# ElementsProject/lightning

Measured on AMD Instinct MI355X. Metric: signature verifies/sec (ECDSA+Schnorr mix), higher is better.
Workload: dtype u32 (256-bit modular integer); 1 GPU; configs[1]+configs[2]: 1000000 ECDSA (65-byte keys, 65536 distinct) + 1000000 BIP-340 Schnorr per GPU per step, 90% valid / 10% invalid, inputs resident in HBM; parallelism=shard-by-row x1, RCCL all-gather of verdicts, key_table_cache=off (tables rebuilt every call)

## Files before the change

lightning_amd/csrc/engine_internal.h:

```cpp
#pragma once
#include <hip/hip_runtime.h>
#include <type_traits>
#include <stdio.h>
#include <stdlib.h>
#include <string.h>

#include <map>
#include <mutex>
#include <random>
#include <string>
#include <atomic>
#include <thread>
#include <vector>

#include "../../include/lightning_amd.h"
#include "../../include/lightning_amd_debug.h"
#include "verify_core.h"

using namespace lamd;

constexpr int MAX_LANES = 8;
#ifndef LAMD_PRIO_DEFAULT
#define LAMD_PRIO_DEFAULT 13
#endif
// ... 56 lines not shown
    for (auto &e : ev) {
      if (e) (void)hipEventDestroy(e);
      e = nullptr;
    }
  }
};

enum { Q_ECDSA33 = 0, Q_ECDSA65 = 1, Q_SCHNORR = 2, Q_KINDS = 3 };
#ifndef LAMD_QUEUE_SETS
#define LAMD_QUEUE_SETS 9
#endif
constexpr int QUEUE_SETS = LAMD_QUEUE_SETS;

struct lamd_ctx {
  int device = 0;
  int gtable_device = -1;
  hipStream_t stream = nullptr;
  hipDeviceProp_t prop;
  u32 *gtable = nullptr;
  std::string err;
  devbuf recs, qwords, keyok, slots, vbuf;
  devbuf row_ent, kd_table, kd_rep, kd_uid, kd_uniq, kd_count, kd_newent, plan, kt_fin;
  struct shape_ws { devbuf row, ent, slot, qwords, keyok, scratch; } hk[2];
  devbuf list7, list10, listcold, listcold_ok;
  u8 *h_small = nullptr;
  struct tmpl_ws {
    u8 *h = nullptr;
    size_t cap = 0;
  } tmpl;
  devbuf small_done;
  std::vector<u64> small_missed;
  u32 prio_mask = LAMD_PRIO_DEFAULT;
  unsigned spin_us = 2000;
  std::vector<u64> learn_fps;
  devbuf learn_dev;
  bool force_learn = false;
  u32 small_ticket = 0;
  bool small_kernel = true;
  u32 *h_plan = nullptr;
  struct key_cache {
    bool shared = false;
    u32 cap_ent = 0, cap7 = 0, cap10 = 0, index_mask = 0;
    devbuf ents, index, pool7, pool10, counters;
  } cache_store;
  key_cache *cache = nullptr;
  lamd_ctx *root = nullptr;
// ... 6 lines not shown
  int cache_mode = 1;
  size_t cache_keys = (size_t)1 << 20, cache_keys10 = (size_t)1 << 16;
  u32 cache_hwm[3] = {0, 0, 0};
  u32 cache_resets = 0;
  size_t last_hits = 0, last_cold = 0, last_l7 = 0, last_l10 = 0;
  devbuf keyok_row;
  hipStream_t stream2 = nullptr;
  hipStream_t stream3 = nullptr;
  hipEvent_t ev_fork = nullptr, ev_prep = nullptr, ev_cold = nullptr, ev_keys = nullptr, ev_sigs = nullptr;
  bool sigs_pending = false;
  hipEvent_t ev_sigs_wait = nullptr;
  static constexpr int MAX_COPY_STREAMS = 4;
  hipStream_t copy_streams[MAX_COPY_STREAMS] = {nullptr, nullptr, nullptr, nullptr};
  int n_copy_streams = 1;
  bool copy_one = true;
  int copy_events = 0;
  unsigned copy_turn = 0;
  bool use_copy_stream = true;
  int keyed_mode = -1;
  size_t keyed_min_rows = 8192;
  bool early_cold = true;
  bool fused_front = true;
  bool kc_tree = false;
  bool small_fused = true;
  bool last_small_fused = false;
  size_t last_small_n = 0;
  double keyed_min_uses = 6.0;
  double keyed_dense_uses = 48.0;
  int keyed_teeth = 0;
  int last_mode = 0;
  size_t last_n = 0;
  bool last_keyed_call = false;
  devbuf in_a, in_b, in_c, out;
  devbuf g_msgs, g_off, g_ids, g_rowbase, g_hash, g_sig, g_pub, g_malformed, g_ok, g_verdict;
  struct store_ws {
    devbuf img, host, ids, tab, out, rep, pack, dig, rng, rng_out, cmp, cmp_out, dir, sq, sq_out, ts, ts_msg, ts_out, rx, rx_out;
    stage_timer<6> t_audit;
    stage_timer<4> t_rep;
    stage_timer<6> t_dig;
    stage_timer<7> t_rx;
    void destroy_events() { t_audit.destroy(); t_rep.destroy(); t_dig.destroy(); t_rx.destroy(); }
  } store;
  struct text_ws {
    devbuf cols;
    stage_timer<3> t;
    double ms[2] = {0, 0};
// ... 101 lines not shown
```

lightning_amd/csrc/lamd_common.h:

```cpp
#pragma once
#include <stddef.h>
#include <stdint.h>

#if defined(__HIPCC__)
#include <hip/hip_runtime.h>
#define LAMD_HD __host__ __device__ __forceinline__
#define LAMD_HD_NOINLINE __host__ __device__ __noinline__
#else
#define LAMD_HD static inline __attribute__((always_inline))
#define LAMD_HD_NOINLINE static __attribute__((noinline))
#endif

#if defined(LAMD_CHECK_MAG)
#include <assert.h>
#define LAMD_ASSERT(x) assert(x)
#else
#define LAMD_ASSERT(x) ((void)0)
#endif

namespace lamd {
typedef uint32_t u32;
typedef uint64_t u64;
typedef uint8_t u8;
}
```

lightning_amd/csrc/lamd_engine.hip:

```cpp
#include "engine_internal.h"
#include "fuzz.h"
#include "host_ranges.h"
#include "key_column.h"
#include "table_audit.h"

using namespace lamd;

__device__ u32 g_prio;
#define LAMD_PRIO(bit)                                     \
  do {                                                     \
    if (g_prio & (bit)) __builtin_amdgcn_s_setprio(3);     \
  } while (0)


__global__ void __launch_bounds__(256) k_gtable_build(u32 *__restrict__ gtable, const u32 *__restrict__ bases) {
  const size_t idx = (size_t)blockIdx.x * blockDim.x + threadIdx.x;
  if (idx >= GTABLE_ENTRIES) return;
  const u32 w = (u32)(idx >> GTABLE_WINDOW_BITS), d = (u32)(idx & ((1u << GTABLE_WINDOW_BITS) - 1u));
  u32 out[GT_ENTRY_WORDS];
  if (d == 0) {
#pragma unroll
    for (int i = 0; i < GT_ENTRY_WORDS; i++) out[i] = 0;
  } else {
    u32 base[16];
// ... 484 lines not shown
#pragma unroll
  for (int i = 0; i < 8; i++) { qx[i] = qwords[u * 16 + i]; qy[i] = qwords[u * 16 + 8 + i]; }
  kc_prefix<T>(pool + (size_t)slots[u] * kc_stride(T), scratch + u * kc_scratch_words(T), ge_from_words(qx, qy));
}
template <int T>
__global__ void __launch_bounds__(256) k_kc_chain_bwd(const u32 *__restrict__ plan, int which, u32 cap, const u8 *__restrict__ keyok,
                                                      u32 *__restrict__ pool, const u32 *__restrict__ slots, const u32 *__restrict__ scratch) {
  const size_t t = (size_t)blockIdx.x * blockDim.x + threadIdx.x;
  const size_t u = t / kc_nsub(T);
  const u32 nkeys = plan[which] < cap ? plan[which] : cap;
  if (u >= nkeys || !keyok[u]) return;
  kc_chain_bwd<T>(pool + (size_t)slots[u] * kc_stride(T), scratch + u * kc_scratch_words(T), (int)(t % kc_nsub(T)));
}
struct kc_shape_args {
  u32 cap;
  const u32 *hk_row;
  const u32 *hk_ent, *hk_slot;
  u32 *qwords;
  u8 *keyok;
  u32 *scratch;
  u32 *pool;
};
template <int T>
static void launch_keytables(hipStream_t st, const u32 *plan, int which, const kc_shape_args &A) {
  const size_t cap = A.cap, chains = cap * kc_nsub(T);
  hipLaunchKernelGGL((k_kc_bases<T>), dim3((unsigned)((cap + 255) / 256)), dim3(256), 0, st, plan, which, A.cap, A.qwords, A.keyok, A.scratch);
  hipLaunchKernelGGL((k_kc_chain_fwd<T>), dim3((unsigned)((chains + 255) / 256)), dim3(256), 0, st, plan, which, A.cap, A.keyok, A.pool, A.hk_slot, A.scratch);
  hipLaunchKernelGGL((k_kc_prefix<T>), dim3((unsigned)((cap + 255) / 256)), dim3(256), 0, st, plan, which, A.cap, A.qwords, A.keyok, A.pool, A.hk_slot,
                     A.scratch);
  hipLaunchKernelGGL((k_kc_chain_bwd<T>), dim3((unsigned)((chains + 255) / 256)), dim3(256), 0, st, plan, which, A.cap, A.keyok, A.pool, A.hk_slot,
                     A.scratch);
}

template <int T>
__device__ __forceinline__ void keys_bases_body(size_t u, const u32 *__restrict__ plan, int which, const kc_shape_args &A, const u8 *__restrict__ keys,
                                                int keylen, size_t stride) {
  const u32 nkeys = plan[which] < A.cap ? plan[which] : A.cap;
  if (u >= nkeys) return;
  u32 qx[8], qy[8];
  const bool ok = parse_pubkey(keys + stride * (size_t)A.hk_row[u], keylen, qx, qy);
  uint4 *dst = reinterpret_cast<uint4 *>(A.qwords + u * 16);
  dst[0] = make_uint4(qx[0], qx[1], qx[2], qx[3]);
  dst[1] = make_uint4(qx[4], qx[5], qx[6], qx[7]);
  dst[2] = make_uint4(qy[0], qy[1], qy[2], qy[3]);
  dst[3] = make_uint4(qy[4], qy[5], qy[6], qy[7]);
  A.keyok[u] = ok;
  if (ok) kc_bases<T>(A.scratch + u * kc_scratch_words(T), ge_from_words(qx, qy));
}
__global__ void __launch_bounds__(256) k_keys_bases_both(const u32 *__restrict__ plan, unsigned blocks7, kc_shape_args A7, kc_shape_args A10,
                                                         const u8 *__restrict__ keys, int keylen, size_t stride) {
  LAMD_PRIO(8);
  if (blockIdx.x < blocks7) keys_bases_body<7>((size_t)blockIdx.x * blockDim.x + threadIdx.x, plan, P_HK7, A7, keys, keylen, stride);
  else keys_bases_body<10>((size_t)(blockIdx.x - blocks7) * blockDim.x + threadIdx.x, plan, P_HK10, A10, keys, keylen, stride);
}
struct publish_args {
  const u8 *keys;
  int keylen;
  size_t stride;
  u32 lane, seq;
  u64 seed;
  cache_ent *ents;
  u32 *index;
  u32 mask;
  int do_index;
};
template <int T>
__device__ __forceinline__ void kc_finish_body(size_t t, const u32 *__restrict__ plan, int which, const kc_shape_args &A, const publish_args &P) {
  constexpr int NS = kc_nsub(T);
  static_assert(256 % NS == 0, "a key's chains must not straddle blocks");
  const size_t u = t / NS;
  const int sub = (int)(t % NS);
  const u32 nkeys = plan[which] < A.cap ? plan[which] : A.cap;
  const bool live = u < nkeys;
  const bool ok = live && A.keyok[u];
  u32 *tab = ok ? A.pool + (size_t)A.hk_slot[u] * kc_stride(T) : nullptr;
  u32 *scr = A.scratch + u * kc_scratch_words(T);
  if (ok) kc_chain_fwd<T>(tab, scr, sub);
  __syncthreads();
  if (live && sub == 0) {
    if (ok) {
      u32 qx[8], qy[8];
#pragma unroll
      for (int i = 0; i < 8; i++) { qx[i] = A.qwords[u * 16 + i]; qy[i] = A.qwords[u * 16 + 8 + i]; }
      kc_prefix<T>(tab, scr, ge_from_words(qx, qy));
    }
    cache_ent e;
    key_words(e.kw, P.keys + P.stride * (size_t)A.hk_row[u], P.keylen);
    e.meta = (ok ? (u32)T : 0u) | (P.lane << 8);
    e.seq = P.seq;
    e.tabslot = A.hk_slot[u];
    const u32 id = A.hk_ent[u];
    P.ents[id] = e;
    if (P.do_index) {
      __threadfence();
      u32 slot = (u32)key_words_hash(e.kw, P.seed) & P.mask;
      for (;;) {
        if (atomicCAS(&P.index[slot], 0u, id + 1u) == 0u) break;
        slot = (slot + 1u) & P.mask;
      }
    }
  }
  __syncthreads();
  if (ok) kc_chain_bwd<T>(tab, scr, sub);
}
__global__ void __launch_bounds__(256) k_kc_finish_both(const u32 *__restrict__ plan, unsigned blocks7, kc_shape_args A7, kc_shape_args A10, publish_args P) {
  LAMD_PRIO(8);
  if (blockIdx.x < blocks7) kc_finish_body<7>((size_t)blockIdx.x * blockDim.x + threadIdx.x, plan, P_HK7, A7, P);
  else kc_finish_body<10>((size_t)(blockIdx.x - blocks7) * blockDim.x + threadIdx.x, plan, P_HK10, A10, P);
}

template <int T, int KPL>
__device__ __forceinline__ void kc_tree_body(size_t t, const u32 *__restrict__ plan, int which, const kc_shape_args &A, const publish_args &P) {
  const u32 nkeys = plan[which] < A.cap ? plan[which] : A.cap;
  const size_t u0 = t * KPL;
  if (u0 >= nkeys) return;
  kc_tree_keys K;
  ge qs[KPL];
  K.n = 0;
#pragma unroll 1
  for (int k = 0; k < KPL; k++) {
    const size_t u = u0 + k;
    if (u >= nkeys) break;
    const bool ok = A.keyok[u] != 0;
    if (ok) {
      u32 qx[8], qy[8];
#pragma unroll
      for (int i = 0; i < 8; i++) { qx[i] = A.qwords[u * 16 + i]; qy[i] = A.qwords[u * 16 + 8 + i]; }
      qs[K.n] = ge_from_words(qx, qy);
      K.tab[K.n] = A.pool + (size_t)A.hk_slot[u] * kc_stride(T);
      K.scr[K.n] = A.scratch + u * kc_scratch_words(T);
      K.n++;
// ... 412 lines not shown
    HIPCHK(ctx, hipDeviceSynchronize());
    HIPCHK(ctx, hipFree(b->p));
  }
  b->p = nullptr;
  b->cap = 0;
  size_t want = bytes + bytes / 4 + 4096;
  if (hipMalloc(&b->p, want) != hipSuccess) {
    want = bytes;
    hipError_t e = hipMalloc(&b->p, want);
    if (e != hipSuccess) {
      ctx->err = std::string("hipMalloc: ") + hipGetErrorString(e);
      return LAMD_ERR_NOMEM;
    }
  }
  b->cap = want;
  return LAMD_OK;
}

static unsigned careful_grid(const lamd_ctx *ctx, size_t n) {
  const bool flood = ctx->h_plan && ((volatile const u32 *)ctx->h_plan)[P_SUSPECT] > 4096u;
  return flood || blocks_for(n) < 64u ? blocks_for(n) : 64u;
}

static unsigned keyed_grid(size_t n) { return (unsigned)((n + KEYED_THREADS - 1) / KEYED_THREADS); }

static int hw_queues_from_env(void) {
  const char *v = getenv("GPU_MAX_HW_QUEUES");
  return v && *v ? atoi(v) : 0;
}

extern "C" const char *lamd_version(void) { return "lightning_amd 0.1 (gfx950)"; }

extern "C" const char *lamd_last_error(const lamd_ctx *ctx) { return ctx ? ctx->err.c_str() : "no context"; }

static int init_known_answers(lamd_ctx *ctx);
static int cache_alloc(lamd_ctx *owner, lamd_ctx::key_cache *kc, size_t keys7, size_t keys10, bool shared);
static int cache_reset(lamd_ctx *root);

static int create_streams(lamd_ctx *ctx) {
  HIPCHK(ctx, hipStreamCreateWithFlags(&ctx->stream, hipStreamNonBlocking));
  HIPCHK(ctx, hipStreamCreateWithFlags(&ctx->stream2, hipStreamNonBlocking));
  if (!getenv("LAMD_MERGE_SIDE") || atoi(getenv("LAMD_MERGE_SIDE")) != 0) ctx->stream3 = ctx->stream2;
  else HIPCHK(ctx, hipStreamCreateWithFlags(&ctx->stream3, hipStreamNonBlocking));
  HIPCHK(ctx, hipEventCreateWithFlags(&ctx->ev_cold, hipEventDisableTiming));
  HIPCHK(ctx, hipEventCreateWithFlags(&ctx->ev_keys, hipEventDisableTiming));
  HIPCHK(ctx, hipEventCreateWithFlags(&ctx->ev_sigs, hipEventDisableTiming));
// ... 82 lines not shown
  if (!out) return LAMD_ERR_ARG;
  *out = nullptr;
  int count = 0;
  if (hipGetDeviceCount(&count) != hipSuccess || count <= 0) return LAMD_ERR_NO_DEVICE;
  if (device < 0 || device >= count) return LAMD_ERR_ARG;
  lamd_ctx *ctx = new (std::nothrow) lamd_ctx();
  if (!ctx) return LAMD_ERR_NOMEM;
  ctx->device = device;
  *out = ctx;
  HIPCHK(ctx, hipSetDevice(device));
  HIPCHK(ctx, hipGetDeviceProperties(&ctx->prop, device));
  if (strncmp(ctx->prop.gcnArchName, "gfx950", 6) != 0) {
    ctx->err = std::string("unsupported architecture ") + ctx->prop.gcnArchName + " (built for gfx950 only)";
    return LAMD_ERR_NO_DEVICE;
  }
  if (const char *w = getenv("LAMD_ECMULT_WAVES")) ctx->ecmult_waves = atoi(w);
  if (const char *w = getenv("LAMD_PAIRS")) ctx->pairs = atoi(w) != 0;
  if (const char *w = getenv("LAMD_GROUP")) ctx->group_rows = atoi(w) != 0;
  if (const char *w = getenv("LAMD_SPIN_US")) ctx->spin_us = (unsigned)atoi(w);
  if (const char *w = getenv("LAMD_PRIO")) ctx->prio_mask = (u32)atoi(w);
  if (const char *w = getenv("LAMD_FUSED_FRONT")) ctx->fused_front = atoi(w) != 0;
  if (const char *w = getenv("LAMD_EARLY_COLD")) ctx->early_cold = atoi(w) != 0;
  if (const char *w = getenv("LAMD_KC_TREE")) ctx->kc_tree = atoi(w) != 0;
  if (const char *w = getenv("LAMD_PREP_BATCH")) ctx->prep_batch = atoi(w) < 1 ? 1 : (size_t)atoi(w);
  if (const char *w = getenv("LAMD_PREP_MIN_THREADS")) ctx->prep_min_threads = atol(w) < 0 ? 0 : (size_t)atol(w);
  {
    std::random_device rd;
    ctx->hash_seed = ((u64)rd() << 32) ^ (u64)rd() ^ 0x243F6A8885A308D3ULL;
  }
  if (const char *w = getenv("LAMD_CHUNK_ROWS")) ctx->chunk = (size_t)atoll(w) < 4 ? 4 : (size_t)atoll(w);
  if (const char *w = getenv("LAMD_KEYED")) ctx->keyed_mode = atoi(w);
  if (const char *w = getenv("LAMD_KEYED_MIN_USES")) ctx->keyed_min_uses = atof(w);
  if (const char *w = getenv("LAMD_KEYED_DENSE_USES")) ctx->keyed_dense_uses = atof(w);
  if (const char *w = getenv("LAMD_KEYED_TEETH")) ctx->keyed_teeth = atoi(w) == 7 ? 7 : (atoi(w) == 10 ? 10 : 0);
  if (const char *w = getenv("LAMD_KEYED_MIN_ROWS")) ctx->keyed_min_rows = (size_t)atoll(w);
  if (const char *w = getenv("LAMD_SMALL_FUSED")) ctx->small_fused = atoi(w) != 0;
  if (const char *w = getenv("LAMD_CACHE")) ctx->cache_mode = atoi(w) != 0;
  if (const char *w = getenv("LAMD_SMALL_KERNEL")) ctx->small_kernel = atoi(w) != 0;
  if (const char *w = getenv("LAMD_CACHE_KEYS")) ctx->cache_keys = (size_t)atoll(w) < 64 ? 64 : (size_t)atoll(w);
  if (const char *w = getenv("LAMD_CACHE_KEYS10")) ctx->cache_keys10 = (size_t)atoll(w) < 16 ? 16 : (size_t)atoll(w);
  int rc = create_streams(ctx);
  if (rc != LAMD_OK) return rc;
  std::vector<u32> bases(GTABLE_WINDOWS * 16);
  {
    const u32 gx[8] = LAMD_GX, gy[8] = LAMD_GY;
    u32 cur[16];
// ... 521 lines not shown
  const size_t n = c.n;
  lamd_ctx::key_cache *kc = f.kc;
  {
    const size_t words = f.m > n ? f.m : n;
    const unsigned ib = blocks_for(words / 4 + 1);
    hipLaunchKernelGGL(k_call_init, dim3(ib < 2048u ? ib : 2048u), dim3(256), 0, ctx->stream, f.plan, ctx->kd_table.as<u32>(), f.m, ctx->kd_count.as<u32>(), n,
                       f.use_cache ? (u32 *)nullptr : f.row_ent, f.use_cache ? (u32 *)nullptr : f.cc);
  }
  if (f.use_cache && (rc = launch_cache_lookup(ctx, root, c, f)) != LAMD_OK) return rc;
  hipLaunchKernelGGL(k_dedupe_insert_count, dim3(blocks_for(n)), dim3(256), 0, ctx->stream, n, c.d_key, c.keylen, c.keystride, root->hash_seed,
                     (const u32 *)f.row_ent, ctx->kd_table.as<u32>(), (u32)(f.m - 1), ctx->kd_rep.as<u32>(), f.plan, ctx->kd_uniq.as<u32>(), ctx->kd_count.as<u32>());
  launch_classify<true>(ctx, c, f);
  if (c.time_it) HIPCHK(ctx, hipEventRecord(ctx->ev[1], ctx->stream));
  if (ctx->early_cold) {
    hipLaunchKernelGGL(k_partition_cold, dim3(blocks_for(n)), dim3(256), 0, ctx->stream, n, ctx->kd_rep.as<const u32>(), ctx->kd_newent.as<const u32>(), f.plan,
                       f.listcold);
    if ((rc = launch_cold(ctx, c, f.listcold, f.plan, f.fin)) != LAMD_OK) return rc;
    *cold_started = true;
  }
  const bool on7 = f.thr[0] != NO_TABLES, on10 = f.thr[1] != NO_TABLES;
  if (on7 || on10) {
    const kc_shape_args A7 = shape_args(ctx->hk[0], on7 ? f.cap[0] : 0, kc->pool7), A10 = shape_args(ctx->hk[1], on10 ? f.cap[1] : 0, kc->pool10);
    const unsigned kb7 = on7 ? blocks_for(f.cap[0]) : 0u, kb10 = on10 ? blocks_for(f.cap[1]) : 0u;
    hipLaunchKernelGGL(k_keys_bases_both, dim3(kb7 + kb10), dim3(256), 0, ctx->stream, (const u32 *)f.plan, kb7, A7, A10, c.d_key, c.keylen, c.keystride);
    const publish_args P = {c.d_key, c.keylen, c.keystride, (u32)ctx->lane_id, f.seq ? f.seq : 1u, root->hash_seed, kc->ents.as<cache_ent>(), kc->index.as<u32>(),
                            kc->index_mask, (int)f.use_cache};
    if (root->kc_tree) {
      const unsigned tb7 = on7 ? (unsigned)((f.cap[0] + 64 * KC_TREE_KPL7 - 1) / (64 * KC_TREE_KPL7)) : 0u;
      const unsigned tb10 = on10 ? (unsigned)((f.cap[1] + 64 * KC_TREE_KPL10 - 1) / (64 * KC_TREE_KPL10)) : 0u;
      hipLaunchKernelGGL(k_kc_tree_both, dim3(tb7 + tb10), dim3(64), 0, ctx->stream, (const u32 *)f.plan, tb7, A7, A10, P);
    } else {
      const unsigned fb7 = on7 ? blocks_for(f.cap[0] * kc_nsub(7)) : 0u, fb10 = on10 ? blocks_for(f.cap[1] * kc_nsub(10)) : 0u;
      hipLaunchKernelGGL(k_kc_finish_both, dim3(fb7 + fb10), dim3(256), 0, ctx->stream, (const u32 *)f.plan, fb7, A7, A10, P);
    }
  }
  if ((rc = mark_published(ctx, root, f)) != LAMD_OK) return rc;
  auto part = *cold_started ? k_partition<true, true> : k_partition<true, false>;
  hipLaunchKernelGGL(part, dim3(blocks_for(n)), dim3(256), 0, ctx->stream, n, f.row_ent, ctx->kd_rep.as<const u32>(), (const u32 *)nullptr,
                     ctx->kd_newent.as<const u32>(), kc->ents.as<const cache_ent>(), f.plan, f.list7, f.list10, f.listcold, c.keyok_out, c.d_ok, c.d_sig, c.mode);
  return LAMD_OK;
}

static int front_end_legacy(lamd_ctx *ctx, lamd_ctx *root, const chunk_io &c, const front_args &f) {
  int rc;
  const size_t n = c.n;
  lamd_ctx::key_cache *kc = f.kc;
  HIPCHK(ctx, hipMemsetAsync(f.plan, 0, P_WORDS * 4, ctx->stream));
  HIPCHK(ctx, hipMemsetAsync(ctx->kd_table.p, 0, f.m * 4, ctx->stream));
  HIPCHK(ctx, hipMemsetAsync(ctx->kd_count.p, 0, n * 4, ctx->stream));
  if (f.use_cache) {
    if ((rc = launch_cache_lookup(ctx, root, c, f)) != LAMD_OK) return rc;
  } else {
    HIPCHK(ctx, hipMemsetAsync(f.row_ent, 0xFF, n * 4, ctx->stream));
    HIPCHK(ctx, hipMemsetAsync(f.cc, 0, C_WORDS * 4, ctx->stream));
  }
  hipLaunchKernelGGL(k_dedupe_insert, dim3(blocks_for(n)), dim3(256), 0, ctx->stream, n, c.d_key, c.keylen, c.keystride, root->hash_seed, (const u32 *)f.row_ent,
// ... 103 lines not shown
}

static int chunk_partitioned(lamd_ctx *ctx, lamd_ctx *root, const chunk_io &c, bool use_cache, bool small, bool latency_learn) {
  int rc;
  const size_t n = c.n;
  front_args f = {};
  f.use_cache = use_cache;
  table_thresholds(ctx, small, use_cache, latency_learn, f.thr);
  for (int s = 0; s < 2; s++) f.cap[s] = f.thr[s] == NO_TABLES ? 1 : n / f.thr[s] + 1;
  lamd_ctx::key_cache *kc = f.kc = use_cache ? &root->cache_store : &ctx->cache_store;
  if (!use_cache && (rc = cache_alloc(ctx, kc, f.cap[0], f.cap[1], false)) != LAMD_OK) return rc;
  f.m = 4;
  while (f.m < 2 * n) f.m <<= 1;
  if ((rc = ensure(ctx, &ctx->kd_table, f.m * 4)) != LAMD_OK) return rc;
  for (devbuf *b : {&ctx->row_ent, &ctx->kd_rep, &ctx->kd_uid, &ctx->kd_uniq, &ctx->kd_count, &ctx->kd_newent, &ctx->list7, &ctx->list10,
                    &ctx->listcold})
    if ((rc = ensure(ctx, b, n * 4)) != LAMD_OK) return rc;
  for (int s = 0; s < 2; s++) {
    lamd_ctx::shape_ws &w = ctx->hk[s];
    for (devbuf *b : {&w.row, &w.ent, &w.slot})
      if ((rc = ensure(ctx, b, f.cap[s] * 4)) != LAMD_OK) return rc;
    if ((rc = ensure(ctx, &w.qwords, f.cap[s] * 64)) != LAMD_OK) return rc;
    if ((rc = ensure(ctx, &w.keyok, f.cap[s])) != LAMD_OK) return rc;
    if ((rc = ensure(ctx, &w.scratch, f.cap[s] * kc_scratch_words(s ? 10 : 7) * 4)) != LAMD_OK) return rc;
  }
  if ((rc = ensure(ctx, &ctx->plan, P_WORDS * 4)) != LAMD_OK) return rc;
  if (c.mode == MODE_SCHNORR && (rc = ensure(ctx, &ctx->kt_fin, n * (size_t)FIN_WORDS * 4)) != LAMD_OK) return rc;
  f.plan = ctx->plan.as<u32>();
  f.cc = kc->counters.as<u32>();
  f.row_ent = ctx->row_ent.as<u32>();
  f.list7 = ctx->list7.as<u32>();
  f.list10 = ctx->list10.as<u32>();
  f.listcold = ctx->listcold.as<u32>();
  f.fin = c.mode == MODE_SCHNORR ? ctx->kt_fin.as<u32>() : nullptr;
  if (use_cache) {
    f.vis = cache_visibility(root, ctx);
    f.seq = ++root->call_seq;
  }
  f.lf = {nullptr, 0, c.d_key, c.keylen, c.keystride, root->hash_seed, 0xFFFFFFFFu, 0xFFFFFFFFu};
  if (small && use_cache) {
    f.lf.budget7 = kc->cap7 / 2;
    f.lf.budget10 = kc->cap10 / 2;
    if (latency_learn && !ctx->learn_fps.empty()) {
      const size_t nf = ctx->learn_fps.size() < 4096 ? ctx->learn_fps.size() : 4096;
      if ((rc = ensure(ctx, &ctx->learn_dev, nf * 8)) != LAMD_OK) return rc;
      HIPCHK(ctx, hipMemcpyAsync(ctx->learn_dev.p, ctx->learn_fps.data(), nf * 8, hipMemcpyHostToDevice, ctx->stream));
      f.lf.fps = ctx->learn_dev.as<const u64>();
// ... 1213 lines not shown
```

lightning_amd/csrc/verify_core.h:

```cpp
#pragma once
#include "group.h"
#include "scalar.h"
#include "sha256.h"

namespace lamd {

enum { MODE_ECDSA = 0, MODE_SCHNORR = 1, MODE_RECOVER = 2 };

#define LAMD_S30_P {0x3FFFFC2F, 0x3FFFFFFB, 0x3FFFFFFF, 0x3FFFFFFF, 0x3FFFFFFF, 0x3FFFFFFF, 0x3FFFFFFF, 0x3FFFFFFF, 0xFFFF}
LAMD_HD fe fe_inv_var(const fe &a) {
  const int32_t pl[9] = LAMD_S30_P;
  u32 aw[8], w[9];
  fe_to_words(aw, fe_normalize(a));
  s30_inverse(w, aw, pl, 0x2DDACACFu);
  const u32 p32[9] = {0xFFFF85E0u, 0xFFFFFFDFu, 0xFFFFFFFFu, 0xFFFFFFFFu, 0xFFFFFFFFu, 0xFFFFFFFFu, 0xFFFFFFFFu, 0xFFFFFFFFu, 0x1Fu};
  u64 cy = 0;
#pragma unroll
  for (int i = 0; i < 9; i++) {
    cy += (u64)w[i] + p32[i];
    w[i] = (u32)cy;
    cy >>= 32;
  }
  u32 q = w[8];
#pragma unroll
// ... 346 lines not shown
  const fe zi = fe_inv_var(acc.z);
  const fe zi2 = fe_sqr(zi);
  slot_store_fe(out, fe_mul(acc.x, zi2));
  slot_store_fe(out + TW, fe_mul(acc.y, fe_mul(zi2, zi)));
}

constexpr int kc_spacing(int T) { return T == 7 ? 19 : T == 8 ? 17 : T == 9 ? 15 : T == 10 ? 13 : 12; }
constexpr int kc_ne(int T) { return 1 << (T - 1); }
constexpr int KC_SUB_LOG = 4, KC_SUB = 1 << KC_SUB_LOG;
constexpr int kc_nsub(int T) { return kc_ne(T) / KC_SUB; }
constexpr int kc_words(int T) { return (kc_ne(T) + 1) * SLOT_ENTRY_WORDS; }
constexpr int kc_stride(int T) { return kc_words(T) + 16; }
constexpr int KC_P0 = 0, KC_ZB = 27, KC_C = 36;
constexpr int kc_sub_off(int T) { return KC_C + (T - 1) * 18; }
constexpr int KC_SUB_WORDS = 18 + (KC_SUB - 1) * 9;
constexpr int kc_scratch_words(int T) { return kc_sub_off(T) + kc_nsub(T) * KC_SUB_WORDS; }
static_assert(kc_nsub(7) * KC_SUB_WORDS >= 13 * 36 && kc_nsub(8) * KC_SUB_WORDS >= 15 * 36, "stage-1 parking space");

LAMD_HD void store_raw(u32 *dst, const fe &a) {
#pragma unroll
  for (int i = 0; i < 9; i++) dst[i] = a.n[i];
}

template <int T>
LAMD_HD void kc_bases(u32 *scratch, const ge &q) {
  constexpr int D = kc_spacing(T), NPT = 2 * T - 1;
  u32 *tmp = scratch + kc_sub_off(T);
  gej b = gej_from_ge(q);
#pragma unroll 1
  for (int i = 0; i < NPT; i++) {
    store_raw(tmp + i * 36 + 0, b.x);
    store_raw(tmp + i * 36 + 9, b.y);
    store_raw(tmp + i * 36 + 18, fe_norm_weak(b.z));
    if (i == NPT - 1) break;
    const int nd = (i & 1) ? D - 1 : 1;
#pragma unroll 1
    for (int j = 0; j < nd; j++) b = gej_double(b);
  }
  fe acc = fe_set_int(1);
#pragma unroll 1
  for (int i = 0; i < NPT; i++) {
    store_raw(tmp + i * 36 + 27, acc);
    acc = fe_mul(acc, slot_load_raw(tmp + i * 36 + 18));
  }
  store_raw(scratch + KC_ZB, acc);
  fe suffix = fe_set_int(1);
#pragma unroll 1
  for (int i = NPT - 1; i >= 0; i--) {
    const fe ratio = fe_mul(suffix, slot_load_raw(tmp + i * 36 + 27));
    suffix = fe_mul(suffix, slot_load_raw(tmp + i * 36 + 18));
    const fe r2 = fe_sqr(ratio);
    const fe x = fe_mul(slot_load_raw(tmp + i * 36 + 0), r2);
    const fe y = fe_mul(slot_load_raw(tmp + i * 36 + 9), fe_mul(r2, ratio));
    u32 *dst = (i & 1) ? scratch + KC_C + (i >> 1) * 18 : tmp + i * 36;
    store_raw(dst + 0, x);
    store_raw(dst + 9, y);
  }
  gej p;
  p.x = slot_load_raw(tmp + (NPT - 1) * 36 + 0);
  p.y = slot_load_raw(tmp + (NPT - 1) * 36 + 9);
  p.z = fe_set_int(1);
  p.inf = false;
#pragma unroll 1
  for (int i = 0; i < T - 1; i++) {
    ge m;
    m.x = slot_load_raw(tmp + 2 * i * 36 + 0);
    m.y = fe_norm_weak(fe_neg(slot_load_raw(tmp + 2 * i * 36 + 9), 1));
    bool degenerate;
    fe h, rr;
    p = gej_add_ge_core(p, m, &degenerate, &h, &rr);
  }
  store_raw(scratch + KC_P0 + 0, p.x);
  store_raw(scratch + KC_P0 + 9, p.y);
  store_raw(scratch + KC_P0 + 18, fe_norm_weak(p.z));
}
template <int T>
LAMD_HD void kc_chain_fwd(u32 *tab, u32 *scratch, int sub) {
  u32 *sp = scratch + kc_sub_off(T) + sub * KC_SUB_WORDS;
  u32 *ent = tab + sub * KC_SUB * SLOT_ENTRY_WORDS;
  gej p;
  p.x = slot_load_raw(scratch + KC_P0 + 0);
  p.y = slot_load_raw(scratch + KC_P0 + 9);
  p.z = slot_load_raw(scratch + KC_P0 + 18);
  p.inf = false;
  bool degenerate;
  fe h, rr;
#pragma unroll 1
  for (int b = 0; b < T - 1 - KC_SUB_LOG; b++) {
    if ((sub >> b) & 1) {
      ge c;
      c.x = slot_load_raw(scratch + KC_C + (KC_SUB_LOG + b) * 18 + 0);
      c.y = slot_load_raw(scratch + KC_C + (KC_SUB_LOG + b) * 18 + 9);
      p = gej_add_ge_core(p, c, &degenerate, &h, &rr);
      p.z = fe_norm_weak(p.z);
    }
  }
  slot_store_fe(ent + 0, p.x);
  slot_store_fe(ent + ENT_Y, p.y);
#pragma unroll 1
  for (int g = 1; g < KC_SUB; g++) {
    const int c = __builtin_ctz((unsigned)g), gr = g ^ (g >> 1);
    ge pt;
    pt.x = slot_load_raw(scratch + KC_C + c * 18 + 0);
    pt.y = slot_load_raw(scratch + KC_C + c * 18 + 9);
    pt = ge_neg_if(pt, ((gr >> c) & 1) == 0);
    p = gej_add_ge_core(p, pt, &degenerate, &h, &rr);
    slot_store_fe(ent + gr * SLOT_ENTRY_WORDS + 0, p.x);
    slot_store_fe(ent + gr * SLOT_ENTRY_WORDS + ENT_Y, p.y);
    store_raw(sp + 18 + (g - 1) * 9, h);
  }
  store_raw(sp + 0, fe_norm_weak(p.z));
}
template <int T>
LAMD_HD void kc_prefix(u32 *tab, u32 *scratch, const ge &q) {
  constexpr int NS = kc_nsub(T), NE = kc_ne(T);
  u32 *sp = scratch + kc_sub_off(T);
  fe acc = fe_set_int(1);
#pragma unroll 1
  for (int s = 0; s < NS; s++) {
    store_raw(sp + s * KC_SUB_WORDS + 9, acc);
    acc = fe_mul(acc, slot_load_raw(sp + s * KC_SUB_WORDS + 0));
  }
  const fe zc = fe_mul(acc, slot_load_raw(scratch + KC_ZB));
  slot_store_fe(tab + kc_words(T), zc);
  fe suffix = fe_set_int(1);
#pragma unroll 1
  for (int s = NS - 1; s >= 0; s--) {
    const fe ratio = fe_mul(suffix, slot_load_raw(sp + s * KC_SUB_WORDS + 9));
    suffix = fe_mul(suffix, slot_load_raw(sp + s * KC_SUB_WORDS + 0));
    store_raw(sp + s * KC_SUB_WORDS + 9, ratio);
  }
  const u32 betaw[8] = LAMD_BETA;
  const fe z2 = fe_sqr(zc);
  const fe x = fe_mul(q.x, z2);
  u32 *e = tab + NE * SLOT_ENTRY_WORDS;
  slot_store_fe(e + 0, x);
  slot_store_fe(e + ENT_BX, fe_mul(x, fe_from_words(betaw)));
  slot_store_fe(e + ENT_Y, fe_mul(q.y, fe_mul(z2, zc)));
}
template <int T>
LAMD_HD void kc_chain_bwd(u32 *tab, const u32 *scratch, int sub) {
  const u32 betaw[8] = LAMD_BETA;
  const fe beta = fe_from_words(betaw);
  const u32 *sp = scratch + kc_sub_off(T) + sub * KC_SUB_WORDS;
  u32 *ent = tab + sub * KC_SUB * SLOT_ENTRY_WORDS;
  fe rho = slot_load_raw(sp + 9);
#pragma unroll 1
  for (int g = KC_SUB - 1; g >= 0; g--) {
    if (g != KC_SUB - 1) rho = fe_mul(rho, slot_load_raw(sp + 18 + g * 9));
    const int gr = g ^ (g >> 1);
    const fe r2 = fe_sqr(rho);
    const fe x = fe_mul(slot_load_fe(ent + gr * SLOT_ENTRY_WORDS + 0), r2);
    const fe y = fe_mul(slot_load_fe(ent + gr * SLOT_ENTRY_WORDS + ENT_Y), fe_mul(r2, rho));
    slot_store_fe(ent + gr * SLOT_ENTRY_WORDS + 0, x);
    slot_store_fe(ent + gr * SLOT_ENTRY_WORDS + ENT_BX, fe_mul(x, beta));
    slot_store_fe(ent + gr * SLOT_ENTRY_WORDS + ENT_Y, y);
  }
}
template <int T>
LAMD_HD void keytable_build(u32 *tab, u32 *scratch, const ge &q) {
  kc_bases<T>(scratch, q);
  for (int s = 0; s < kc_nsub(T); s++) kc_chain_fwd<T>(tab, scratch, s);
  kc_prefix<T>(tab, scratch, q);
  for (int s = 0; s < kc_nsub(T); s++) kc_chain_bwd<T>(tab, scratch, s);
}

constexpr int KC_TREE_MAXK = 4;
struct kc_tree_keys {
  u32 *tab[KC_TREE_MAXK];
  u32 *scr[KC_TREE_MAXK];
  int n;
};
template <int T>
LAMD_HD void kc_tree_affine(const kc_tree_keys &K, const ge *qs) {
  constexpr int NE = kc_ne(T);
  static_assert(kc_nsub(T) * KC_SUB_WORDS >= (NE / 2) * 9, "prefix products of the last level fit the per-chain scratch");
  const u32 betaw[8] = LAMD_BETA;
  const fe beta = fe_from_words(betaw);
  fe acc = fe_set_int(1);
#pragma unroll 1
// ... 1352 lines not shown
```

Measured before the change: 248.7 million verifies/s.

## Interleave key-table scratch per lane and run table kernels as persistent grids

Key-table scratch moves from a flat per-key layout to a lane-interleaved layout of 16-byte chunks, so neighbouring threads' loads and stores coalesce. The chain kernel now parks intermediate points in a per-block chain buffer instead of writing them to the table and reading them back. Both table kernels become grid-stride loops over groups, sized by a grid that defaults to the CU count and can be set with LAMD_TABLE_GRID. The publish step also hashes key words while writing them in place. The catch is extra scratch memory and a bigger chunk footprint (9-word elements padded to 12), and the smaller grid may cut parallelism if one block per CU cannot hide latency.

```diff
diff --git a/lightning_amd/csrc/engine_internal.h b/lightning_amd/csrc/engine_internal.h
--- a/lightning_amd/csrc/engine_internal.h
+++ b/lightning_amd/csrc/engine_internal.h
@@ -102,6 +102,7 @@
   devbuf recs, qwords, keyok, slots, vbuf;
   devbuf row_ent, kd_table, kd_rep, kd_uid, kd_uniq, kd_count, kd_newent, plan, kt_fin;
   struct shape_ws { devbuf row, ent, slot, qwords, keyok, scratch; } hk[2];
+  devbuf kc_chains;
   devbuf list7, list10, listcold, listcold_ok;
   u8 *h_small = nullptr;
   struct tmpl_ws {
@@ -154,6 +155,7 @@
   bool early_cold = true;
   bool fused_front = true;
   bool kc_tree = false;
+  unsigned table_grid = 0;
   bool small_fused = true;
   bool last_small_fused = false;
   size_t last_small_n = 0;
diff --git a/lightning_amd/csrc/lamd_common.h b/lightning_amd/csrc/lamd_common.h
--- a/lightning_amd/csrc/lamd_common.h
+++ b/lightning_amd/csrc/lamd_common.h
@@ -6,9 +6,11 @@
 #include <hip/hip_runtime.h>
 #define LAMD_HD __host__ __device__ __forceinline__
 #define LAMD_HD_NOINLINE __host__ __device__ __noinline__
+#define LAMD_HD_MEMBER __host__ __device__ __forceinline__
 #else
 #define LAMD_HD static inline __attribute__((always_inline))
 #define LAMD_HD_NOINLINE static __attribute__((noinline))
+#define LAMD_HD_MEMBER inline __attribute__((always_inline))
 #endif
 
 #if defined(LAMD_CHECK_MAG)
diff --git a/lightning_amd/csrc/lamd_engine.hip b/lightning_amd/csrc/lamd_engine.hip
--- a/lightning_amd/csrc/lamd_engine.hip
+++ b/lightning_amd/csrc/lamd_engine.hip
@@ -530,6 +530,10 @@
   u32 *pool;
 };
 template <int T>
+__device__ __forceinline__ kc_lanes kc_key_view(u32 *scratch, size_t u) {
+  return kc_lanes{scratch + (u / 64u) * (size_t)(64 * 4 * kc_key_chunks(T)), 64, u % 64u};
+}
+template <int T>
 static void launch_keytables(hipStream_t st, const u32 *plan, int which, const kc_shape_args &A) {
   const size_t cap = A.cap, chains = cap * kc_nsub(T);
   hipLaunchKernelGGL((k_kc_bases<T>), dim3((unsigned)((cap + 255) / 256)), dim3(256), 0, st, plan, which, A.cap, A.qwords, A.keyok, A.scratch);
@@ -540,10 +544,8 @@
                      A.scratch);
 }
 
-template <int T>
-__device__ __forceinline__ void keys_bases_body(size_t u, const u32 *__restrict__ plan, int which, const kc_shape_args &A, const u8 *__restrict__ keys,
-                                                int keylen, size_t stride) {
-  const u32 nkeys = plan[which] < A.cap ? plan[which] : A.cap;
+template <int T, bool LANES>
+__device__ __forceinline__ void keys_bases_body(size_t u, u32 nkeys, const kc_shape_args &A, const u8 *__restrict__ keys, int keylen, size_t stride) {
   if (u >= nkeys) return;
   u32 qx[8], qy[8];
   const bool ok = parse_pubkey(keys + stride * (size_t)A.hk_row[u], keylen, qx, qy);
@@ -553,13 +555,22 @@
   dst[2] = make_uint4(qy[0], qy[1], qy[2], qy[3]);
   dst[3] = make_uint4(qy[4], qy[5], qy[6], qy[7]);
   A.keyok[u] = ok;
-  if (ok) kc_bases<T>(A.scratch + u * kc_scratch_words(T), ge_from_words(qx, qy));
-}
-__global__ void __launch_bounds__(256) k_keys_bases_both(const u32 *__restrict__ plan, unsigned blocks7, kc_shape_args A7, kc_shape_args A10,
-                                                         const u8 *__restrict__ keys, int keylen, size_t stride) {
+  if (!ok) return;
+  if constexpr (LANES) kc_bases_at<T>(kc_key_view<T>(A.scratch, u), ge_from_words(qx, qy));
+  else kc_bases<T>(A.scratch + u * kc_scratch_words(T), ge_from_words(qx, qy));
+}
+template <bool LANES>
+__global__ void __launch_bounds__(256) k_keys_bases_both(const u32 *__restrict__ plan, kc_shape_args A7, kc_shape_args A10, const u8 *__restrict__ keys,
+                                                         int keylen, size_t stride) {
   LAMD_PRIO(8);
-  if (blockIdx.x < blocks7) keys_bases_body<7>((size_t)blockIdx.x * blockDim.x + threadIdx.x, plan, P_HK7, A7, keys, keylen, stride);
-  else keys_bases_body<10>((size_t)(blockIdx.x - blocks7) * blockDim.x + threadIdx.x, plan, P_HK10, A10, keys, keylen, stride);
+  const u32 n7 = plan[P_HK7] < A7.cap ? plan[P_HK7] : A7.cap, n10 = plan[P_HK10] < A10.cap ? plan[P_HK10] : A10.cap;
+  const u32 groups7 = (n7 + 63u) / 64u, groups = groups7 + (n10 + 63u) / 64u;
+  const u32 lane = threadIdx.x & 63u, waves = gridDim.x * (blockDim.x / 64u);
+#pragma unroll 1
+  for (u32 g = blockIdx.x * (blockDim.x / 64u) + threadIdx.x / 64u; g < groups; g += waves) {
+    if (g < groups7) keys_bases_body<7, LANES>((size_t)g * 64u + lane, n7, A7, keys, keylen, stride);
+    else keys_bases_body<10, LANES>((size_t)(g - groups7) * 64u + lane, n10, A10, keys, keylen, stride);
+  }
 }
 struct publish_args {
   const u8 *keys;
@@ -572,36 +583,52 @@
   u32 mask;
   int do_index;
 };
+__device__ __forceinline__ u64 publish_key_words(cache_ent *dst, const u8 *p, int len, u64 seed) {
+  u64 h = seed;
+  u32 even = 0;
+#pragma unroll 1
+  for (int w = 0; w < 17; w++) {
+    u32 v = 0;
+    for (int b = 0; b < 4; b++) {
+      const int k = 4 * w + b;
+      if (k < len) v |= (u32)p[k] << (8 * b);
+    }
+    if (w == 16) v |= (u32)len << 8;
+    dst->kw[w] = v;
+    if (w == 16) h = splitmix64(h ^ v);
+    else if (w & 1) h = splitmix64(h ^ ((u64)even | ((u64)v << 32)));
+    else even = v;
+  }
+  return h;
+}
 template <int T>
-__device__ __forceinline__ void kc_finish_body(size_t t, const u32 *__restrict__ plan, int which, const kc_shape_args &A, const publish_args &P) {
+__device__ __forceinline__ void kc_finish_body(size_t t, u32 nkeys, const kc_shape_args &A, const publish_args &P, const kc_lanes &chain) {
   constexpr int NS = kc_nsub(T);
   static_assert(256 % NS == 0, "a key's chains must not straddle blocks");
   const size_t u = t / NS;
   const int sub = (int)(t % NS);
-  const u32 nkeys = plan[which] < A.cap ? plan[which] : A.cap;
   const bool live = u < nkeys;
   const bool ok = live && A.keyok[u];
   u32 *tab = ok ? A.pool + (size_t)A.hk_slot[u] * kc_stride(T) : nullptr;
-  u32 *scr = A.scratch + u * kc_scratch_words(T);
-  if (ok) kc_chain_fwd<T>(tab, scr, sub);
+  const kc_lanes key = kc_key_view<T>(A.scratch, u);
+  if (ok) kc_chain_fwd_at<T>(tab, key, chain, sub);
   __syncthreads();
   if (live && sub == 0) {
     if (ok) {
       u32 qx[8], qy[8];
 #pragma unroll
       for (int i = 0; i < 8; i++) { qx[i] = A.qwords[u * 16 + i]; qy[i] = A.qwords[u * 16 + 8 + i]; }
-      kc_prefix<T>(tab, scr, ge_from_words(qx, qy));
-    }
-    cache_ent e;
-    key_words(e.kw, P.keys + P.stride * (size_t)A.hk_row[u], P.keylen);
-    e.meta = (ok ? (u32)T : 0u) | (P.lane << 8);
-    e.seq = P.seq;
-    e.tabslot = A.hk_slot[u];
+      kc_prefix_at<T>(tab, key, chain, ge_from_words(qx, qy));
+    }
     const u32 id = A.hk_ent[u];
-    P.ents[id] = e;
+    cache_ent *const e = P.ents + id;
+    const u64 hash = publish_key_words(e, P.keys + P.stride * (size_t)A.hk_row[u], P.keylen, P.seed);
+    e->meta = (ok ? (u32)T : 0u) | (P.lane << 8);
+    e->seq = P.seq;
+    e->tabslot = A.hk_slot[u];
     if (P.do_index) {
       __threadfence();
-      u32 slot = (u32)key_words_hash(e.kw, P.seed) & P.mask;
+      u32 slot = (u32)hash & P.mask;
       for (;;) {
         if (atomicCAS(&P.index[slot], 0u, id + 1u) == 0u) break;
         slot = (slot + 1u) & P.mask;
@@ -609,12 +636,18 @@
     }
   }
   __syncthreads();
-  if (ok) kc_chain_bwd<T>(tab, scr, sub);
-}
-__global__ void __launch_bounds__(256) k_kc_finish_both(const u32 *__restrict__ plan, unsigned blocks7, kc_shape_args A7, kc_shape_args A10, publish_args P) {
+  if (ok) kc_chain_bwd_at<T>(tab, chain, sub);
+}
+__global__ void __launch_bounds__(256) k_kc_finish_both(const u32 *__restrict__ plan, kc_shape_args A7, kc_shape_args A10, publish_args P, u32 *chains) {
   LAMD_PRIO(8);
-  if (blockIdx.x < blocks7) kc_finish_body<7>((size_t)blockIdx.x * blockDim.x + threadIdx.x, plan, P_HK7, A7, P);
-  else kc_finish_body<10>((size_t)(blockIdx.x - blocks7) * blockDim.x + threadIdx.x, plan, P_HK10, A10, P);
+  const kc_lanes chain = {chains + (size_t)blockIdx.x * (256 * 4 * KC_CHAIN_CHUNKS), 256, threadIdx.x};
+  const u32 n7 = plan[P_HK7] < A7.cap ? plan[P_HK7] : A7.cap, n10 = plan[P_HK10] < A10.cap ? plan[P_HK10] : A10.cap;
+  const u64 groups7 = ((u64)n7 * kc_nsub(7) + 255u) / 256u, groups = groups7 + ((u64)n10 * kc_nsub(10) + 255u) / 256u;
+#pragma unroll 1
+  for (u64 g = blockIdx.x; g < groups; g += gridDim.x) {
+    if (g < groups7) kc_finish_body<7>((size_t)g * 256u + threadIdx.x, n7, A7, P, chain);
+    else kc_finish_body<10>((size_t)(g - groups7) * 256u + threadIdx.x, n10, A10, P, chain);
+  }
 }
 
 template <int T, int KPL>
@@ -1073,6 +1106,11 @@
   return flood || blocks_for(n) < 64u ? blocks_for(n) : 64u;
 }
 
+static unsigned table_grid(const lamd_ctx *root, unsigned bound) {
+  const unsigned want = root->table_grid ? root->table_grid : (unsigned)root->prop.multiProcessorCount;
+  return want < bound ? (want ? want : 1u) : bound;
+}
+
 static unsigned keyed_grid(size_t n) { return (unsigned)((n + KEYED_THREADS - 1) / KEYED_THREADS); }
 
 static int hw_queues_from_env(void) {
@@ -1201,6 +1239,7 @@
   if (const char *w = getenv("LAMD_FUSED_FRONT")) ctx->fused_front = atoi(w) != 0;
   if (const char *w = getenv("LAMD_EARLY_COLD")) ctx->early_cold = atoi(w) != 0;
   if (const char *w = getenv("LAMD_KC_TREE")) ctx->kc_tree = atoi(w) != 0;
+  if (const char *w = getenv("LAMD_TABLE_GRID")) ctx->table_grid = atoi(w) < 0 ? 0u : (unsigned)atoi(w);
   if (const char *w = getenv("LAMD_PREP_BATCH")) ctx->prep_batch = atoi(w) < 1 ? 1 : (size_t)atoi(w);
   if (const char *w = getenv("LAMD_PREP_MIN_THREADS")) ctx->prep_min_threads = atol(w) < 0 ? 0 : (size_t)atol(w);
   {
@@ -1768,7 +1807,7 @@
   if (on7 || on10) {
     const kc_shape_args A7 = shape_args(ctx->hk[0], on7 ? f.cap[0] : 0, kc->pool7), A10 = shape_args(ctx->hk[1], on10 ? f.cap[1] : 0, kc->pool10);
     const unsigned kb7 = on7 ? blocks_for(f.cap[0]) : 0u, kb10 = on10 ? blocks_for(f.cap[1]) : 0u;
-    hipLaunchKernelGGL(k_keys_bases_both, dim3(kb7 + kb10), dim3(256), 0, ctx->stream, (const u32 *)f.plan, kb7, A7, A10, c.d_key, c.keylen, c.keystride);
+    hipLaunchKernelGGL(root->kc_tree ? k_keys_bases_both<false> : k_keys_bases_both<true>, dim3(table_grid(root, kb7 + kb10)), dim3(256), 0, ctx->stream, (const u32 *)f.plan, A7, A10, c.d_key, c.keylen, c.keystride);
     const publish_args P = {c.d_key, c.keylen, c.keystride, (u32)ctx->lane_id, f.seq ? f.seq : 1u, root->hash_seed, kc->ents.as<cache_ent>(), kc->index.as<u32>(),
                             kc->index_mask, (int)f.use_cache};
     if (root->kc_tree) {
@@ -1777,7 +1816,9 @@
       hipLaunchKernelGGL(k_kc_tree_both, dim3(tb7 + tb10), dim3(64), 0, ctx->stream, (const u32 *)f.plan, tb7, A7, A10, P);
     } else {
       const unsigned fb7 = on7 ? blocks_for(f.cap[0] * kc_nsub(7)) : 0u, fb10 = on10 ? blocks_for(f.cap[1] * kc_nsub(10)) : 0u;
-      hipLaunchKernelGGL(k_kc_finish_both, dim3(fb7 + fb10), dim3(256), 0, ctx->stream, (const u32 *)f.plan, fb7, A7, A10, P);
+      const unsigned fgrid = table_grid(root, fb7 + fb10);
+      if ((rc = ensure(ctx, &ctx->kc_chains, (size_t)fgrid * 256 * KC_CHAIN_CHUNKS * 16)) != LAMD_OK) return rc;
+      hipLaunchKernelGGL(k_kc_finish_both, dim3(fgrid), dim3(256), 0, ctx->stream, (const u32 *)f.plan, A7, A10, P, ctx->kc_chains.as<u32>());
     }
   }
   if ((rc = mark_published(ctx, root, f)) != LAMD_OK) return rc;
@@ -1927,7 +1968,8 @@
       if ((rc = ensure(ctx, b, f.cap[s] * 4)) != LAMD_OK) return rc;
     if ((rc = ensure(ctx, &w.qwords, f.cap[s] * 64)) != LAMD_OK) return rc;
     if ((rc = ensure(ctx, &w.keyok, f.cap[s])) != LAMD_OK) return rc;
-    if ((rc = ensure(ctx, &w.scratch, f.cap[s] * kc_scratch_words(s ? 10 : 7) * 4)) != LAMD_OK) return rc;
+    const size_t flat = f.cap[s] * kc_scratch_words(s ? 10 : 7) * 4, groups = (f.cap[s] + 63) / 64 * (size_t)(64 * 16 * kc_key_chunks(s ? 10 : 7));
+    if ((rc = ensure(ctx, &w.scratch, flat > groups ? flat : groups)) != LAMD_OK) return rc;
   }
   if ((rc = ensure(ctx, &ctx->plan, P_WORDS * 4)) != LAMD_OK) return rc;
   if (c.mode == MODE_SCHNORR && (rc = ensure(ctx, &ctx->kt_fin, n * (size_t)FIN_WORDS * 4)) != LAMD_OK) return rc;
diff --git a/lightning_amd/csrc/verify_core.h b/lightning_amd/csrc/verify_core.h
--- a/lightning_amd/csrc/verify_core.h
+++ b/lightning_amd/csrc/verify_core.h
@@ -392,16 +392,73 @@
   for (int i = 0; i < 9; i++) dst[i] = a.n[i];
 }
 
-template <int T>
-LAMD_HD void kc_bases(u32 *scratch, const ge &q) {
+struct alignas(16) kc_chunk { u32 w[4]; };
+constexpr int KC_SLOT_CHUNKS = 3, KC_PARK_CHUNKS = (TW + 3) / 4;
+constexpr int kc_key_slots(int T) { return 4 + 2 * (T - 1); }
+constexpr int KC_CHAIN_SLOTS = 2 + (KC_SUB - 1);
+static_assert(kc_key_slots(7) * 9 == kc_sub_off(7) && kc_key_slots(10) * 9 == kc_sub_off(10) && KC_CHAIN_SLOTS * 9 == KC_SUB_WORDS, "slots of the flat layout");
+constexpr int kc_key_chunks(int T) { return (kc_key_slots(T) + 4 * (2 * T - 1)) * KC_SLOT_CHUNKS; }
+constexpr int KC_CHAIN_CHUNKS = KC_CHAIN_SLOTS * KC_SLOT_CHUNKS + 2 * KC_SUB * KC_PARK_CHUNKS;
+struct kc_flat {
+  u32 *p;
+  static constexpr bool parks = false;
+  LAMD_HD_MEMBER fe load(int s) const { return slot_load_raw(p + 9 * s); }
+  LAMD_HD_MEMBER void store(int s, const fe &a) const { store_raw(p + 9 * s, a); }
+  LAMD_HD_MEMBER kc_flat after(int slots) const { return kc_flat{p + 9 * slots}; }
+  LAMD_HD_MEMBER kc_flat chain(int s) const { return kc_flat{p + s * KC_SUB_WORDS}; }
+  LAMD_HD_MEMBER fe unpark(int) const { return fe_set_int(0); }
+  LAMD_HD_MEMBER void park(int, const fe &) const {}
+};
+struct kc_lanes {
+  u32 *base;
+  size_t stride, lane;
+  static constexpr bool parks = true;
+  LAMD_HD_MEMBER kc_chunk *chunk(int c) const { return reinterpret_cast<kc_chunk *>(base + ((size_t)c * stride + lane) * 4); }
+  LAMD_HD_MEMBER fe load(int s) const {
+    const kc_chunk a = *chunk(3 * s), b = *chunk(3 * s + 1);
+    fe r;
+#pragma unroll
+    for (int i = 0; i < 4; i++) { r.n[i] = a.w[i]; r.n[4 + i] = b.w[i]; }
+    r.n[8] = chunk(3 * s + 2)->w[0];
+    FE_SETMAG(r, 1);
+    return r;
+  }
+  LAMD_HD_MEMBER void store(int s, const fe &a) const {
+    *chunk(3 * s) = kc_chunk{{a.n[0], a.n[1], a.n[2], a.n[3]}};
+    *chunk(3 * s + 1) = kc_chunk{{a.n[4], a.n[5], a.n[6], a.n[7]}};
+    *chunk(3 * s + 2) = kc_chunk{{a.n[8], 0, 0, 0}};
+  }
+  LAMD_HD_MEMBER kc_lanes after(int slots) const { return kc_lanes{base + (size_t)slots * KC_SLOT_CHUNKS * stride * 4, stride, lane}; }
+  LAMD_HD_MEMBER kc_lanes chain(int s) const { return kc_lanes{base, stride, lane + (size_t)s}; }
+  LAMD_HD_MEMBER void park(int k, const fe &a) const {
+    u32 w[4 * KC_PARK_CHUNKS] = {};
+    slot_store_fe(w, a);
+#pragma unroll
+    for (int c = 0; c < KC_PARK_CHUNKS; c++)
+      *chunk(KC_CHAIN_SLOTS * KC_SLOT_CHUNKS + k * KC_PARK_CHUNKS + c) = kc_chunk{{w[4 * c], w[4 * c + 1], w[4 * c + 2], w[4 * c + 3]}};
+  }
+  LAMD_HD_MEMBER fe unpark(int k) const {
+    u32 w[4 * KC_PARK_CHUNKS];
+#pragma unroll
+    for (int c = 0; c < KC_PARK_CHUNKS; c++) {
+      const kc_chunk v = *chunk(KC_CHAIN_SLOTS * KC_SLOT_CHUNKS + k * KC_PARK_CHUNKS + c);
+#pragma unroll
+      for (int i = 0; i < 4; i++) w[4 * c + i] = v.w[i];
+    }
+    return slot_load_fe(w);
+  }
+};
+
+template <int T, class K>
+LAMD_HD void kc_bases_at(const K &key, const ge &q) {
   constexpr int D = kc_spacing(T), NPT = 2 * T - 1;
-  u32 *tmp = scratch + kc_sub_off(T);
+  const K tmp = key.after(kc_key_slots(T));
   gej b = gej_from_ge(q);
 #pragma unroll 1
   for (int i = 0; i < NPT; i++) {
-    store_raw(tmp + i * 36 + 0, b.x);
-    store_raw(tmp + i * 36 + 9, b.y);
-    store_raw(tmp + i * 36 + 18, fe_norm_weak(b.z));
+    tmp.store(i * 4 + 0, b.x);
+    tmp.store(i * 4 + 1, b.y);
+    tmp.store(i * 4 + 2, fe_norm_weak(b.z));
     if (i == NPT - 1) break;
     const int nd = (i & 1) ? D - 1 : 1;
 #pragma unroll 1
@@ -410,48 +467,51 @@
   fe acc = fe_set_int(1);
 #pragma unroll 1
   for (int i = 0; i < NPT; i++) {
-    store_raw(tmp + i * 36 + 27, acc);
-    acc = fe_mul(acc, slot_load_raw(tmp + i * 36 + 18));
-  }
-  store_raw(scratch + KC_ZB, acc);
+    tmp.store(i * 4 + 3, acc);
+    acc = fe_mul(acc, tmp.load(i * 4 + 2));
+  }
+  key.store(3, acc);
   fe suffix = fe_set_int(1);
 #pragma unroll 1
   for (int i = NPT - 1; i >= 0; i--) {
-    const fe ratio = fe_mul(suffix, slot_load_raw(tmp + i * 36 + 27));
-    suffix = fe_mul(suffix, slot_load_raw(tmp + i * 36 + 18));
+    const fe ratio = fe_mul(suffix, tmp.load(i * 4 + 3));
+    suffix = fe_mul(suffix, tmp.load(i * 4 + 2));
     const fe r2 = fe_sqr(ratio);
-    const fe x = fe_mul(slot_load_raw(tmp + i * 36 + 0), r2);
-    const fe y = fe_mul(slot_load_raw(tmp + i * 36 + 9), fe_mul(r2, ratio));
-    u32 *dst = (i & 1) ? scratch + KC_C + (i >> 1) * 18 : tmp + i * 36;
-    store_raw(dst + 0, x);
-    store_raw(dst + 9, y);
+    const fe x = fe_mul(tmp.load(i * 4 + 0), r2);
+    const fe y = fe_mul(tmp.load(i * 4 + 1), fe_mul(r2, ratio));
+    if (i & 1) {
+      key.store(4 + (i >> 1) * 2, x);
+      key.store(5 + (i >> 1) * 2, y);
+    } else {
+      tmp.store(i * 4 + 0, x);
+      tmp.store(i * 4 + 1, y);
+    }
   }
   gej p;
-  p.x = slot_load_raw(tmp + (NPT - 1) * 36 + 0);
-  p.y = slot_load_raw(tmp + (NPT - 1) * 36 + 9);
+  p.x = tmp.load((NPT - 1) * 4 + 0);
+  p.y = tmp.load((NPT - 1) * 4 + 1);
   p.z = fe_set_int(1);
   p.inf = false;
 #pragma unroll 1
   for (int i = 0; i < T - 1; i++) {
     ge m;
-    m.x = slot_load_raw(tmp + 2 * i * 36 + 0);
-    m.y = fe_norm_weak(fe_neg(slot_load_raw(tmp + 2 * i * 36 + 9), 1));
+    m.x = tmp.load(2 * i * 4 + 0);
+    m.y = fe_norm_weak(fe_neg(tmp.load(2 * i * 4 + 1), 1));
     bool degenerate;
     fe h, rr;
     p = gej_add_ge_core(p, m, &degenerate, &h, &rr);
   }
-  store_raw(scratch + KC_P0 + 0, p.x);
-  store_raw(scratch + KC_P0 + 9, p.y);
-  store_raw(scratch + KC_P0 + 18, fe_norm_weak(p.z));
-}
-template <int T>
-LAMD_HD void kc_chain_fwd(u32 *tab, u32 *scratch, int sub) {
-  u32 *sp = scratch + kc_sub_off(T) + sub * KC_SUB_WORDS;
+  key.store(0, p.x);
+  key.store(1, p.y);
+  key.store(2, fe_norm_weak(p.z));
+}
+template <int T, class K, class C>
+LAMD_HD void kc_chain_fwd_at(u32 *tab, const K &key, const C &sp, int sub) {
   u32 *ent = tab + sub * KC_SUB * SLOT_ENTRY_WORDS;
   gej p;
-  p.x = slot_load_raw(scratch + KC_P0 + 0);
-  p.y = slot_load_raw(scratch + KC_P0 + 9);
-  p.z = slot_load_raw(scratch + KC_P0 + 18);
+  p.x = key.load(0);
+  p.y = key.load(1);
+  p.z = key.load(2);
   p.inf = false;
   bool degenerate;
   fe h, rr;
@@ -459,46 +519,55 @@
   for (int b = 0; b < T - 1 - KC_SUB_LOG; b++) {
     if ((sub >> b) & 1) {
       ge c;
-      c.x = slot_load_raw(scratch + KC_C + (KC_SUB_LOG + b) * 18 + 0);
-      c.y = slot_load_raw(scratch + KC_C + (KC_SUB_LOG + b) * 18 + 9);
+      c.x = key.load(4 + (KC_SUB_LOG + b) * 2);
+      c.y = key.load(5 + (KC_SUB_LOG + b) * 2);
       p = gej_add_ge_core(p, c, &degenerate, &h, &rr);
       p.z = fe_norm_weak(p.z);
     }
   }
-  slot_store_fe(ent + 0, p.x);
-  slot_store_fe(ent + ENT_Y, p.y);
+  if constexpr (C::parks) {
+    sp.park(0, p.x);
+    sp.park(1, p.y);
+  } else {
+    slot_store_fe(ent + 0, p.x);
+    slot_store_fe(ent + ENT_Y, p.y);
+  }
 #pragma unroll 1
   for (int g = 1; g < KC_SUB; g++) {
     const int c = __builtin_ctz((unsigned)g), gr = g ^ (g >> 1);
     ge pt;
-    pt.x = slot_load_raw(scratch + KC_C + c * 18 + 0);
-    pt.y = slot_load_raw(scratch + KC_C + c * 18 + 9);
+    pt.x = key.load(4 + c * 2);
+    pt.y = key.load(5 + c * 2);
     pt = ge_neg_if(pt, ((gr >> c) & 1) == 0);
     p = gej_add_ge_core(p, pt, &degenerate, &h, &rr);
-    slot_store_fe(ent + gr * SLOT_ENTRY_WORDS + 0, p.x);
-    slot_store_fe(ent + gr * SLOT_ENTRY_WORDS + ENT_Y, p.y);
-    store_raw(sp + 18 + (g - 1) * 9, h);
-  }
-  store_raw(sp + 0, fe_norm_weak(p.z));
-}
-template <int T>
-LAMD_HD void kc_prefix(u32 *tab, u32 *scratch, const ge &q) {
+    if constexpr (C::parks) {
+      sp.park(2 * gr, p.x);
+      sp.park(2 * gr + 1, p.y);
+    } else {
+      slot_store_fe(ent + gr * SLOT_ENTRY_WORDS + 0, p.x);
+      slot_store_fe(ent + gr * SLOT_ENTRY_WORDS + ENT_Y, p.y);
+    }
+    sp.store(1 + g, h);
+  }
+  sp.store(0, fe_norm_weak(p.z));
+}
+template <int T, class K, class C>
+LAMD_HD void kc_prefix_at(u32 *tab, const K &key, const C &sp, const ge &q) {
   constexpr int NS = kc_nsub(T), NE = kc_ne(T);
-  u32 *sp = scratch + kc_sub_off(T);
   fe acc = fe_set_int(1);
 #pragma unroll 1
   for (int s = 0; s < NS; s++) {
-    store_raw(sp + s * KC_SUB_WORDS + 9, acc);
-    acc = fe_mul(acc, slot_load_raw(sp + s * KC_SUB_WORDS + 0));
-  }
-  const fe zc = fe_mul(acc, slot_load_raw(scratch + KC_ZB));
+    sp.chain(s).store(1, acc);
+    acc = fe_mul(acc, sp.chain(s).load(0));
+  }
+  const fe zc = fe_mul(acc, key.load(3));
   slot_store_fe(tab + kc_words(T), zc);
   fe suffix = fe_set_int(1);
 #pragma unroll 1
   for (int s = NS - 1; s >= 0; s--) {
-    const fe ratio = fe_mul(suffix, slot_load_raw(sp + s * KC_SUB_WORDS + 9));
-    suffix = fe_mul(suffix, slot_load_raw(sp + s * KC_SUB_WORDS + 0));
-    store_raw(sp + s * KC_SUB_WORDS + 9, ratio);
+    const fe ratio = fe_mul(suffix, sp.chain(s).load(1));
+    suffix = fe_mul(suffix, sp.chain(s).load(0));
+    sp.chain(s).store(1, ratio);
   }
   const u32 betaw[8] = LAMD_BETA;
   const fe z2 = fe_sqr(zc);
@@ -508,24 +577,33 @@
   slot_store_fe(e + ENT_BX, fe_mul(x, fe_from_words(betaw)));
   slot_store_fe(e + ENT_Y, fe_mul(q.y, fe_mul(z2, zc)));
 }
-template <int T>
-LAMD_HD void kc_chain_bwd(u32 *tab, const u32 *scratch, int sub) {
+template <int T, class C>
+LAMD_HD void kc_chain_bwd_at(u32 *tab, const C &sp, int sub) {
   const u32 betaw[8] = LAMD_BETA;
   const fe beta = fe_from_words(betaw);
-  const u32 *sp = scratch + kc_sub_off(T) + sub * KC_SUB_WORDS;
   u32 *ent = tab + sub * KC_SUB * SLOT_ENTRY_WORDS;
-  fe rho = slot_load_raw(sp + 9);
+  fe rho = sp.load(1);
 #pragma unroll 1
   for (int g = KC_SUB - 1; g >= 0; g--) {
-    if (g != KC_SUB - 1) rho = fe_mul(rho, slot_load_raw(sp + 18 + g * 9));
+    if (g != KC_SUB - 1) rho = fe_mul(rho, sp.load(2 + g));
     const int gr = g ^ (g >> 1);
     const fe r2 = fe_sqr(rho);
-    const fe x = fe_mul(slot_load_fe(ent + gr * SLOT_ENTRY_WORDS + 0), r2);
-    const fe y = fe_mul(slot_load_fe(ent + gr * SLOT_ENTRY_WORDS + ENT_Y), fe_mul(r2, rho));
+    const fe x = fe_mul(C::parks ? sp.unpark(2 * gr) : slot_load_fe(ent + gr * SLOT_ENTRY_WORDS + 0), r2);
+    const fe y = fe_mul(C::parks ? sp.unpark(2 * gr + 1) : slot_load_fe(ent + gr * SLOT_ENTRY_WORDS + ENT_Y), fe_mul(r2, rho));
     slot_store_fe(ent + gr * SLOT_ENTRY_WORDS + 0, x);
     slot_store_fe(ent + gr * SLOT_ENTRY_WORDS + ENT_BX, fe_mul(x, beta));
     slot_store_fe(ent + gr * SLOT_ENTRY_WORDS + ENT_Y, y);
   }
+}
+template <int T>
+LAMD_HD void kc_bases(u32 *scratch, const ge &q) { kc_bases_at<T>(kc_flat{scratch}, q); }
+template <int T>
+LAMD_HD void kc_chain_fwd(u32 *tab, u32 *scratch, int sub) { kc_chain_fwd_at<T>(tab, kc_flat{scratch}, kc_flat{scratch + kc_sub_off(T)}.chain(sub), sub); }
+template <int T>
+LAMD_HD void kc_prefix(u32 *tab, u32 *scratch, const ge &q) { kc_prefix_at<T>(tab, kc_flat{scratch}, kc_flat{scratch + kc_sub_off(T)}, q); }
+template <int T>
+LAMD_HD void kc_chain_bwd(u32 *tab, const u32 *scratch, int sub) {
+  kc_chain_bwd_at<T>(tab, kc_flat{const_cast<u32 *>(scratch) + kc_sub_off(T)}.chain(sub), sub);
 }
 template <int T>
 LAMD_HD void keytable_build(u32 *tab, u32 *scratch, const ge &q) {
```

Result: faster. 256.6 million verifies/s (median of 6 runs) (+3.2%).
